# speechcatcher-asr/speechcatcher

Hardware: AMD Instinct MI355X
Metric: concurrent real-time streams (audio-seconds/s), de_xl dims, 640 ms (10240-sample) chunk steps, beam 10 CTC+attention (higher is better)
Workload: dtype f32

## Files before the change

include/scasr.h:

```cpp
#ifndef SCASR_H
#define SCASR_H

#include <stddef.h>
#include <stdint.h>

#ifdef __cplusplus
extern "C" {
#endif

#define SC_OK 0
#define SC_ERR_ARG (-1)
#define SC_ERR_LAUNCH (-2)
#define SC_ERR_CAPACITY (-3)
#define SC_ERR_INPUT (-4)

#define SC_GEMM_RELU 1
#define SC_GEMM_RESIDUAL 2
#define SC_GEMM_LN_AT_CROWS 8
#define SC_GEMM_NAIVE 4
#define SC_GEMM_SPLIT16 16

#define SC_F_ANY_EOS 1
#define SC_F_BEST_EOS 2
#define SC_F_ALL_EOS 4
// ... 494 lines not shown
int sc_conv1(const float *feat, int n_mels, const int32_t *jobs, int n_jobs, int max_t1,
             const float *w, const float *b, int d, float *c1, void *stream);

int sc_block_pack(const float *sub, const int32_t *jobs, int nb, int R, const float *pe, int d,
                  float *xblk, void *stream);

int sc_ctx_handoff(float *x, int R, const int32_t *jobs, int ns, float *state, int layer, int d,
                   void *stream);

int sc_enc_attention(const float *qkv, float *att, int nblk, int R, int H, int d, int masked,
                     void *stream);

int sc_encoder_layers(const sc_enc_layer *layers , int n_layers, float *x, int nblk, int R,
                      int masked, const int32_t *jobs, int ns, float *past_ctx, float *xn,
                      float *qkv, float *att, float *ffh, int d, int H, int F, float eps,
                      void *stream);


int sc_ctc_extend_state(const sc_search *sb , void *stream);
int sc_dec_embed(const sc_search *sb, void *stream);
int sc_kv_rows_to_half(const float *stage, const int32_t *rows, int m, int n_layers, int TCAP, int d2,
                       void *ckv_half, void *stream);
int sc_dec_self_attn(const sc_search *sb, int layer, void *stream);
int sc_dec_cross_attn(const sc_search *sb, int layer, void *stream);
int sc_decoder_layers(const sc_search *sb, void *stream);
#define SC_MAX_VOCAB 8192
int sc_logsoftmax_topk(const sc_search *sb, void *stream);
int sc_ctc_prefix_scan(const sc_search *sb, void *stream);
int sc_ctc_prefix_scan_split(const sc_search *sb, int split_min, void *stream);
int sc_fuse_topw(const sc_search *sb, void *stream);
int sc_beam_prune(const sc_search *sb, void *stream);
int sc_ctc_gather_state(const sc_search *sb, void *stream);
int sc_ctc_gather_state_split(const sc_search *sb, int split_min, void *stream);
int sc_decode_step(const sc_search *sb, void *stream);
int sc_decode_step_ex(const sc_search *sb, int scan_split_min, void *stream);
int sc_dec_layer_fused_supported(int d, int H, int W, int F);
int sc_dec_layer_self(const sc_search *sb, int layer, const float *x_in, float *x_out, const float *ffn_part,
                      int n_ffn_part, void *stream);
int sc_dec_layer_cross(const sc_search *sb, int layer, const float *x_in, float *x_out, void *stream);
int sc_dec_layer_ffn(const sc_search *sb, int layer, const float *x_in, float *x_out, float *ffn_part,
                     int max_part, int *n_part , void *stream);
int sc_dec_layer_stream_supported(int d, int H, int W, int F);
int sc_dec_layer_stream(const sc_search *sb, int layer, const float *x_in, float *x_out, float *xn_out,
                        const float *ffn_part, int n_ffn_part, void *stream);
int sc_dec_layer_ffn_xn(const sc_search *sb, int layer, const float *xn, float *ffn_part, int max_part,
                        int *n_part , void *stream);
int sc_dec_layer_reduce_ln(const sc_search *sb, int layer, const float *x_in, float *x_out, float *xn_out, void *stream);
int sc_dec_output_logits(const sc_search *sb, const float *x_in, float *x_out, const float *ffn_part,
                         int n_ffn_part, void *stream);


int sc_glu_dwconv_bn_swish(const float *y, int B, int T, int C, int ksize, const float *dw_w,
                           const float *dw_b, const float *bn_g, const float *bn_b,
                           const float *bn_mean, const float *bn_var, float bn_eps, float *out,
                           void *stream);

int sc_relpos_attention(const float *qkv, const float *p, const float *bias_u, const float *bias_v,
                        float *out, int B, int T, int H, int d, void *stream);
int sc_relpos_attention_masked(const float *qkv, const float *p, const float *bias_u, const float *bias_v,
                               float *out, int B, int T, int H, int d, const uint8_t *mask, int mask_mode,
                               void *stream);

typedef struct sc_config {
  int32_t d_model, enc_heads, enc_layers, dec_heads, dec_layers, ffn_dim, vocab_size;
  int32_t n_mels, n_fft, win_length, hop_length, sample_rate;
  int32_t block_size, hop_size, look_ahead, subsample, conv_freq1, conv_freq2;
// ... 135 lines not shown
```

speechcatcher_amd/_abi.py:

```python
import ctypes as C
import os
import subprocess
from pathlib import Path

HERE = Path(__file__).resolve().parent
LIB_PATH = HERE / "libscasr.so"
CSRC = HERE / "csrc"

c_float_p = C.POINTER(C.c_float)
c_int_p = C.POINTER(C.c_int32)
c_double_p = C.POINTER(C.c_double)
vp = C.c_void_p


class EncLayer(C.Structure):
    _fields_ = [(n, vp) for n in ("ln1_g", "ln1_b", "wqkv", "bqkv", "wo", "bo",
                                  "ln2_g", "ln2_b", "w1", "b1", "w2", "b2", "w1_p", "w2_p",
                                  "wqkv_p", "wo_p", "w1_h", "w2_h", "wqkv_h", "wo_h", "w1_s", "w2_s",
                                  "wqkv_s", "wo_s")]


class DecLayer(C.Structure):
    _fields_ = [(n, vp) for n in ("ln1_g", "ln1_b", "wqkv", "bqkv", "wo", "bo",
                                  "ln2_g", "ln2_b", "wq", "bq", "wo2", "bo2",
# ... 258 lines not shown
    "sc_prof_collect": (C.c_int, [c_double_p, c_double_p, C.POINTER(C.c_longlong)]),
    "sc_prof_collect2": (C.c_int, [c_double_p, c_double_p, c_double_p, C.POINTER(C.c_longlong)]),
    "sc_prof_event_overhead_ms": (C.c_double, [vp]),
    "sc_layernorm": (C.c_int, [vp, vp, C.c_int, vp, vp, C.c_int, C.c_int, C.c_int, vp, vp, C.c_float, vp]),
    "sc_copy_rows": (C.c_int, [vp, vp, vp, vp, C.c_int, C.c_int, vp]),
    "sc_log_softmax_rows": (C.c_int, [vp, vp, C.c_int, C.c_int, vp]),
    "sc_logmel": (C.c_int, [vp, C.c_int, vp, C.c_int, C.c_int, vp, vp, vp, vp, vp, C.c_int, C.c_int,
                            C.c_int, C.c_int, C.c_int, vp, vp]),
    "sc_conv1": (C.c_int, [vp, C.c_int, vp, C.c_int, C.c_int, vp, vp, C.c_int, vp, vp]),
    "sc_block_pack": (C.c_int, [vp, vp, C.c_int, C.c_int, vp, C.c_int, vp, vp]),
    "sc_ctx_handoff": (C.c_int, [vp, C.c_int, vp, C.c_int, vp, C.c_int, C.c_int, vp]),
    "sc_enc_attention": (C.c_int, [vp, vp, C.c_int, C.c_int, C.c_int, C.c_int, C.c_int, vp]),
    "sc_encoder_layers": (C.c_int, [vp, C.c_int, vp, C.c_int, C.c_int, C.c_int, vp, C.c_int, vp, vp,
                                    vp, vp, vp, C.c_int, C.c_int, C.c_int, C.c_float, vp]),
    "sc_glu_dwconv_bn_swish": (C.c_int, [vp, C.c_int, C.c_int, C.c_int, C.c_int, vp, vp, vp, vp, vp, vp,
                                         C.c_float, vp, vp]),
    "sc_relpos_attention": (C.c_int, [vp, vp, vp, vp, vp, C.c_int, C.c_int, C.c_int, C.c_int, vp]),
    "sc_relpos_attention_masked": (C.c_int, [vp, vp, vp, vp, vp, C.c_int, C.c_int, C.c_int, C.c_int, vp, C.c_int, vp]),
    "sc_ctc_extend_state": (C.c_int, [vp, vp]),
    "sc_dec_embed": (C.c_int, [vp, vp]),
    "sc_kv_rows_to_half": (C.c_int, [vp, vp, C.c_int, C.c_int, C.c_int, C.c_int, vp, vp]),
    "sc_dec_self_attn": (C.c_int, [vp, C.c_int, vp]),
    "sc_dec_cross_attn": (C.c_int, [vp, C.c_int, vp]),
    "sc_decoder_layers": (C.c_int, [vp, vp]),
    "sc_logsoftmax_topk": (C.c_int, [vp, vp]),
    "sc_ctc_prefix_scan": (C.c_int, [vp, vp]),
    "sc_fuse_topw": (C.c_int, [vp, vp]),
    "sc_beam_prune": (C.c_int, [vp, vp]),
    "sc_ctc_gather_state": (C.c_int, [vp, vp]),
    "sc_ctc_gather_state_split": (C.c_int, [vp, C.c_int, vp]),
    "sc_decode_step": (C.c_int, [vp, vp]),
    "sc_decode_step_ex": (C.c_int, [vp, C.c_int, vp]),
    "sc_ctc_prefix_scan_split": (C.c_int, [vp, C.c_int, vp]),
    "sc_dec_layer_fused_supported": (C.c_int, [C.c_int, C.c_int, C.c_int, C.c_int]),
    "sc_dec_layer_self": (C.c_int, [vp, C.c_int, vp, vp, vp, C.c_int, vp]),
    "sc_dec_layer_cross": (C.c_int, [vp, C.c_int, vp, vp, vp]),
    "sc_dec_layer_ffn": (C.c_int, [vp, C.c_int, vp, vp, vp, C.c_int, C.POINTER(C.c_int), vp]),
    "sc_dec_output_logits": (C.c_int, [vp, vp, vp, vp, C.c_int, vp]),
    "sc_streams_kv_rows": (C.c_int, [vp]),
    "sc_dec_layer_stream_supported": (C.c_int, [C.c_int, C.c_int, C.c_int, C.c_int]),
    "sc_dec_layer_stream": (C.c_int, [vp, C.c_int, vp, vp, vp, vp, C.c_int, vp]),
    "sc_dec_layer_reduce_ln": (C.c_int, [vp, C.c_int, vp, vp, vp, vp]),
    "sc_dec_layer_ffn_xn": (C.c_int, [vp, C.c_int, vp, vp, C.c_int, C.POINTER(C.c_int), vp]),
    "sc_engine_create": (C.c_int, [C.POINTER(Config), C.POINTER(NamedTensor), C.c_int, C.c_int, C.POINTER(vp)]),
    "sc_engine_load": (C.c_int, [C.c_char_p, C.c_int, C.POINTER(vp)]),
    "sc_engine_config": (C.c_int, [vp, C.POINTER(Config)]),
    "sc_engine_destroy": (None, [vp]),
    "sc_streams_create": (C.c_int, [vp, C.POINTER(StreamOptions), C.POINTER(vp)]),
    "sc_streams_destroy": (None, [vp]),
    "sc_push": (C.c_int, [vp, c_int_p, C.POINTER(vp), c_int_p, C.POINTER(C.c_uint8), C.c_int, c_int_p]),
    "sc_push_features": (C.c_int, [vp, c_int_p, C.POINTER(vp), c_int_p, C.POINTER(C.c_uint8), C.c_int, c_int_p]),
    "sc_get_hyps": (C.c_int, [vp, C.c_int, C.c_int, C.c_int, c_int_p, c_int_p, c_int_p, c_double_p, c_double_p,
                              c_double_p]),
    "sc_get_hyps_batch": (C.c_int, [vp, c_int_p, C.c_int, C.c_int, C.c_int, c_int_p, c_int_p, c_int_p, c_int_p,
                                    c_double_p, c_double_p, c_double_p]),
    "sc_submit": (C.c_int, [vp, c_int_p, C.POINTER(vp), c_int_p, C.POINTER(C.c_uint8), C.c_int]),
    "sc_poll": (C.c_int, [vp, C.c_int, C.c_int, c_int_p, c_int_p]),
    "sc_streams_outstanding": (C.c_int, [vp]),
    "sc_streams_set_encoder_batch": (C.c_int, [vp, C.c_int]),
    "sc_streams_set_queue_depth": (C.c_int, [vp, C.c_int]),
    "sc_stream_last_error": (C.c_char_p, [vp, C.c_int]),
    "sc_reset": (C.c_int, [vp, C.c_int]),
    "sc_stream_info": (C.c_int, [vp, C.c_int, C.POINTER(StreamInfo)]),
    "sc_streams_stats": (C.c_int, [vp, C.POINTER(C.c_long), C.POINTER(C.c_long), C.POINTER(C.c_long)]),
    "sc_streams_capture_stats": (C.c_int, [vp, C.POINTER(C.c_long), c_double_p]),
    "sc_streams_set_graphs": (C.c_int, [vp, C.c_int]),
# ... 138 lines not shown
```

speechcatcher_amd/csrc/search.hip:

```cpp
#include "common.h"
#include "attn.h"
#include <mutex>
#include <unordered_map>

#define SC_CTC_T(s) (CTRL(s, SC_C_TCTC) > 0 ? CTRL(s, SC_C_TCTC) : CTRL(s, SC_C_T))

#define XPOS(pp, s, h) (sb.xpos + (((long)(pp) * sb.S + (s)) * sb.W + (h)) * sb.LCAP)
#define CTCR(pp, s) (sb.ctc_r + ((long)(pp) * sb.S + (s)) * sb.TCAP * 2 * sb.W)
#define CTCRS(pp, s) (sb.ctc_rs + ((long)(pp) * sb.S + (s)) * sb.TCAP * sb.W)

__global__ void ctc_extend_state_kernel(sc_search sb) {
  const int s = blockIdx.x, h = threadIdx.x;
  if (!CTRL(s, SC_C_ACTIVE) || !CTRL(s, SC_C_HAS)) return;
  const int T = CTRL(s, SC_C_T), told = CTRL(s, SC_C_TOLD), nh = CTRL(s, SC_C_NHYP);
  if (h >= nh || told >= T) return;
  float *r = CTCR(CTRL(s, SC_C_CUR), s);
  float *rs = CTCRS(CTRL(s, SC_C_CUR), s);
  const float *x = sb.ctcx + (long)s * sb.TCAP * sb.V;
  const int t0 = told < 1 ? 1 : told;
  float rb = r[((long)(t0 - 1) * 2 + 1) * sb.W + h];
  for (int t = t0; t < T; ++t) {
    rb = rb + x[(long)t * sb.V + sb.blank];
    r[((long)t * 2 + 0) * sb.W + h] = SC_LOGZERO;
    r[((long)t * 2 + 1) * sb.W + h] = rb;
// ... 573 lines not shown
    float phi;
    ctc_frame(r_n, r_b, prs, pb, same, xc, xb, phi);
    if ((i & (SC_CTC_CK - 1)) == SC_CTC_CK - 1) {
      rn[((long)(t / SC_CTC_CK) * 2) * WK + e] = r_n;
      rn[((long)(t / SC_CTC_CK) * 2 + 1) * WK + e] = r_b;
    }
    ctc_psi_add(pm, ps, phi + xc);
    if (!has) cum += xb;
  };
  auto advance = [&](const CtcChunkT &q, int tb) {
    if (tb >= start && tb + 16 <= T) {
#pragma unroll
      for (int i = 0; i < 16; ++i) frame(q, tb, i);
    } else {
#pragma unroll
      for (int i = 0; i < 16; ++i)
        if (tb + i >= start && tb + i < T) frame(q, tb, i);
    }
  };
  if (start < T) {
    CtcChunkT qa, qb;
    int tb = start & ~15;
    fetch(qa, tb);
    while (true) {
      if (tb + 16 < T) fetch(qb, tb + 16);
      advance(qa, tb);
      tb += 16;
      if (tb >= T) break;
      if (tb + 16 < T) fetch(qa, tb + 16);
      advance(qb, tb);
      tb += 16;
      if (tb >= T) break;
    }
  }
  float psi = pm + logf(ps);
  const float rsum_last = has ? rsp[(long)(T - 1) * W + h] : cum;
  if (c == sb.eos) psi = rsum_last;
  if (c == sb.blank) psi = SC_LOGZERO;
  sb.psi[row * K + k] = psi;
  if (k == 0) sb.psi_eos[row] = rsum_last;
}

#define CTC_EB (256 / CTC_NSEG)
__global__ __launch_bounds__(256) void ctc_prefix_scan_tpar_kernel(sc_search sb, int split_min) {
  __shared__ float co[8][CTC_NSEG][CTC_EB];
  __shared__ float st0[2][CTC_NSEG][CTC_EB];
  __shared__ float cum0[CTC_NSEG][CTC_EB];
  const int s = blockIdx.y;
  if (!CTRL(s, SC_C_ACTIVE)) return;
  const int nh = CTRL(s, SC_C_NHYP), K = sb.K, W = sb.W, V = sb.V;
  const int T = SC_CTC_T(s), L = CTRL(s, SC_C_L), cur = CTRL(s, SC_C_CUR);
  if (!ctc_scan_is_split(T, L, split_min)) return;
  if ((int)blockIdx.x * CTC_EB >= nh * K) return;
  const int el = threadIdx.x % CTC_EB, p = threadIdx.x / CTC_EB;
  const int e_raw = blockIdx.x * CTC_EB + el;
  const bool valid = e_raw < nh * K;
  const int e = valid ? e_raw : nh * K - 1;
  const int h = e / K, k = e % K;
  const bool has = CTRL(s, SC_C_HAS);
  const long row = (long)s * W + h;
  const int c = sb.pre_ids[row * K + k];
  const int last = YSEQ(cur, s, h)[L - 1];
  const bool same = (c == last);
  const int tct = sb.tct;
  const float *__restrict__ xcol = sb.ctcxT + ((long)s * V + c) * tct;
  const float *__restrict__ xblk = sb.ctcxT + ((long)s * V + sb.blank) * tct;
// ... 91 lines not shown
    float n = r_n0, b = r_b0;
    float gm = r_n0, gs = 1.f;
    for (int q = 0; q < CTC_NSEG; ++q) {
      st0[0][q][el] = n;
      st0[1][q][el] = b;
      const float nn = lse2(co[0][q][el] + n, co[3][q][el]);
      const float nb = lse2(lse2(co[1][q][el] + n, co[2][q][el] + b), co[4][q][el]);
      n = nn;
      b = nb;
      const float m = sc_max_raw(gm, co[5][q][el]);
      gs = gs * sc_exp_neg(gm - m) + co[6][q][el] * sc_exp_neg(co[5][q][el] - m);
      gm = m;
    }
    if (valid) {
      float psi = gm + logf(gs);
      float total = 0.f;
      if (!has)
        for (int q = 0; q < CTC_NSEG; ++q) total += co[7][q][el];
      const float rsum_last = has ? rsp[(long)(T - 1) * W + h] : total;
      if (c == sb.eos) psi = rsum_last;
      if (c == sb.blank) psi = SC_LOGZERO;
      sb.psi[row * K + k] = psi;
      if (k == 0) sb.psi_eos[row] = rsum_last;
    }
  }
  __syncthreads();
  if (valid) {
    rn[((long)p * 2) * WK + e] = st0[0][p][el];
    rn[((long)p * 2 + 1) * WK + e] = st0[1][p][el];
  }
}

static std::mutex g_scan_split_mutex;
static std::unordered_map<const void *, int> g_scan_split;
static void scan_split_note(const sc_search *sbp, int eff) {
  std::lock_guard<std::mutex> lk(g_scan_split_mutex);
  g_scan_split[sbp->ctc_rnew] = eff;
}
static int scan_split_last(const sc_search *sbp) {
  std::lock_guard<std::mutex> lk(g_scan_split_mutex);
  auto it = g_scan_split.find(sbp->ctc_rnew);
  return it == g_scan_split.end() ? -1 : it->second;
}

extern "C" int sc_ctc_prefix_scan_split(const sc_search *sbp, int split_min, void *stream) {
  SC_CHECK_ARG(sbp, "null");
  SC_CHECK_ARG(sbp->ctcxT && sbp->tct >= 4 && sbp->tct % 4 == 0, "the prefix scan needs the column-major table copy (sc_search.ctcxT)");
  split_min = ctc_split_min_ok(sbp->TCAP, split_min);
  scan_split_note(sbp, split_min);
  dim3 grid(cdiv(sbp->W * sbp->K, 256), sbp->S);
  ctc_prefix_scan_colmajor_kernel<<<grid, 256, 0, (hipStream_t)stream>>>(*sbp, split_min);
  if (split_min > 0)
    ctc_prefix_scan_tpar_kernel<<<dim3(cdiv(sbp->W * sbp->K, CTC_EB), sbp->S), 256, 0, (hipStream_t)stream>>>(*sbp, split_min);
  SC_CHECK_LAUNCH();
  return SC_OK;
}

extern "C" int sc_ctc_prefix_scan(const sc_search *sbp, void *stream) { return sc_ctc_prefix_scan_split(sbp, 0, stream); }

__device__ __forceinline__ float sort_key_value(unsigned long long c) {
  unsigned u = (unsigned)(c >> 32);
  u = (u & 0x80000000u) ? (u & 0x7FFFFFFFu) : ~u;
  return __uint_as_float(u);
}

__global__ __launch_bounds__(256) void fuse_topw_kernel(sc_search sb) {
  extern __shared__ __attribute__((aligned(16))) float smem[];
  __shared__ int need_full;
  const int row = blockIdx.x, s = row / sb.W, h = row % sb.W;
  if (!CTRL(s, SC_C_ACTIVE) || h >= CTRL(s, SC_C_NHYP)) return;
  const int V = sb.V, K = sb.K, W = sb.W, tid = threadIdx.x;
  float *comb = smem, *ctc = smem + V;
  if (!(sb.w_ctc > 0.f)) {
    if (tid < W) {
      const int c = sb.pre_ids[(long)row * K + tid];
      sb.cand_tok[(long)row * W + tid] = c;
      sb.cand_score[(long)row * W + tid] = __fmul_rn(sb.w_dec, sb.logp[(long)row * V + c]);
      sb.cand_ctc[(long)row * W + tid] = 0.f;
    }
    return;
  }
  const float s_prev = CTRL(s, SC_C_HAS) ? sb.ctc_s[((long)CTRL(s, SC_C_CUR) * sb.S + s) * W + h] : 0.f;
  if (K < 64 && W <= 64 && sb.w_dec >= 0.f) {
    if (tid < 64) {
// ... 40 lines not shown
  }
  __syncthreads();
  for (int v = tid; v < V; v += 256) {
    const float cv = __fsub_rn(ctc[v], s_prev);
    ctc[v] = cv;
    comb[v] = __fadd_rn(__fmul_rn(sb.w_dec, sb.logp[(long)row * V + v]), __fmul_rn(sb.w_ctc, cv));
  }
  __syncthreads();
  const int NP = next_pow2(V);
  unsigned long long *comp = reinterpret_cast<unsigned long long *>(smem + 2 * V);
  for (int c = tid; c < NP; c += 256) comp[c] = c < V ? sort_key(comb[c], c) : 0ull;
  __syncthreads();
  block_bitonic_sort_desc(comp, NP);
  for (int k = tid; k < W; k += 256) {
    const int i = sort_key_index(comp[k]);
    sb.cand_tok[(long)row * W + k] = i;
    sb.cand_score[(long)row * W + k] = comb[i];
    sb.cand_ctc[(long)row * W + k] = ctc[i];
  }
}

extern "C" int sc_fuse_topw(const sc_search *sbp, void *stream) {
  SC_CHECK_ARG(sbp, "null");
  SC_CHECK_ARG(sbp->V > 0 && sbp->V <= SC_MAX_VOCAB, "vocabulary larger than SC_MAX_VOCAB (8192)");
  const size_t smem = fuse_topw_lds(sbp->V);
  const int rc = allow_large_lds(reinterpret_cast<const void *>(&fuse_topw_kernel), smem, fuse_topw_lds(SC_MAX_VOCAB),
                                 "sc_fuse_topw");
  if (rc != SC_OK) return rc;
  fuse_topw_kernel<<<sbp->S * sbp->W, 256, smem, (hipStream_t)stream>>>(*sbp);
  SC_CHECK_LAUNCH();
  return SC_OK;
}

__global__ __launch_bounds__(256) void beam_prune_kernel(sc_search sb) {
  extern __shared__ __attribute__((aligned(16))) double tot[];
  __shared__ int fl_any, fl_all, fl_best, fl_rep;
  __shared__ int win_h[64], win_tok[64];
  __shared__ unsigned bm[SC_KV_MAX_ROWS / 32];
  const int s = blockIdx.x, tid = threadIdx.x;
  if (!CTRL(s, SC_C_ACTIVE)) return;
  for (int w = tid; w < (sb.kv_rows + 31) / 32; w += 256) bm[w] = 0u;
  const int W = sb.W, K = sb.K;
  const int nh = CTRL(s, SC_C_NHYP), L = CTRL(s, SC_C_L), T = CTRL(s, SC_C_T);
  const int cur = CTRL(s, SC_C_CUR), o = 1 - cur;
  const int n = nh * W, nout = n < W ? n : W;
  if (tid == 0) { fl_any = 0; fl_all = 1; fl_best = 0; fl_rep = 0; }
  for (int e = tid; e < n; e += 256) {
    const int h = e / W, j = e % W;
    tot[e] = sb.score[((long)cur * sb.S + s) * W + h] + (double)sb.cand_score[((long)s * W + h) * W + j];
  }
  __syncthreads();
  for (int e = tid; e < n; e += 256) {
    const double te = tot[e];
    int rk = 0;
    for (int j = 0; j < n; ++j) rk += (tot[j] > te) || (tot[j] == te && j < e);
    if (rk >= nout) continue;
    const int h = e / W, j = e % W, i = rk;
    const long prow = (long)s * W + h;
    const int tok = sb.cand_tok[prow * W + j];
    win_h[i] = h;
    win_tok[i] = tok;
    const long oi = ((long)o * sb.S + s) * W + i, ci = ((long)cur * sb.S + s) * W + h;
    sb.score[oi] = te;
    sb.sc_dec[oi] = sb.sc_dec[ci] + (double)sb.logp[prow * sb.V + tok];
    sb.sc_ctc[oi] = sb.sc_ctc[ci] + (double)sb.cand_ctc[prow * W + j];
    int kk = -1;
    for (int q = 0; q < K; ++q)
      if (sb.pre_ids[prow * K + q] == tok) { kk = q; break; }
    float sval;
    if (tok == sb.blank) sval = SC_LOGZERO;
    else if (tok == sb.eos) sval = sb.psi_eos[prow];
    else if (kk >= 0) sval = sb.psi[prow * K + kk];
    else sval = SC_LOGZERO;
    sb.ctc_s[oi] = sval;
    sb.sel[((long)s * W + i) * 2] = h;
    sb.sel[((long)s * W + i) * 2 + 1] = kk < 0 ? 0 : kk;
    const bool is_eos = tok == sb.eos;
    if (is_eos) atomicOr(&fl_any, 1);
    else atomicAnd(&fl_all, 0);
    if (i == 0 && is_eos) atomicOr(&fl_best, 1);
  }
  __syncthreads();
  const int *asrc = ANC(cur, s);
  int *adst = ANC(o, s);
  bool rep = false;
  constexpr int UB = 4;
  const int ntot = nout * (L + 1);
  for (int e0 = tid; e0 < ntot; e0 += 256 * UB) {
    int yv[UB], xv[UB], av[UB];
#pragma unroll
    for (int u = 0; u < UB; ++u) {
      const int e = min(e0 + 256 * u, ntot - 1);
      const int i = e / (L + 1), p = min(e % (L + 1), L - 1);
      const int h = win_h[i];
      yv[u] = YSEQ(cur, s, h)[p];
      xv[u] = XPOS(cur, s, h)[p];
      av[u] = asrc[(long)p * W + h];
    }
#pragma unroll
    for (int u = 0; u < UB; ++u) {
      const int e = e0 + 256 * u;
      if (e >= ntot) break;
      const int i = e / (L + 1), p = e % (L + 1);
      const int tok = win_tok[i];
      int *ydst = YSEQ(o, s, i), *xdst = XPOS(o, s, i);
      if (p < L) {
        ydst[p] = yv[u];
        xdst[p] = xv[u];
        if (p >= 1 && yv[u] == tok && tok != sb.sos && tok != sb.eos) rep = true;
        adst[(long)p * W + i] = av[u];
        atomicOr(&bm[(av[u] >> 5) & (SC_KV_MAX_ROWS / 32 - 1)], 1u << (av[u] & 31));
      } else {
        ydst[L] = tok;
        xdst[L] = T - 1;
      }
    }
  }
  if (rep) atomicOr(&fl_rep, 1);
  __syncthreads();
  if (tid == 0)
    sb.flags[s] = (fl_any ? SC_F_ANY_EOS : 0) | (fl_best ? SC_F_BEST_EOS : 0) |
                  (fl_all ? SC_F_ALL_EOS : 0) | (fl_rep ? SC_F_REPEAT : 0);
  if (tid >= 64 || L + 1 > sb.LCAP) return;
  const int lane = tid, NR = sb.kv_rows, nwords = (NR + 31) / 32;
  int *out = adst + (long)L * W;
  int got = 0;
  for (int w0 = 0; w0 < nwords && got < nout; w0 += 64) {
    const int w = w0 + lane;
    unsigned fr = w < nwords ? ~bm[w] : 0u;
    if (w == nwords - 1 && (NR & 31)) fr &= (1u << (NR & 31)) - 1u;
    const int c = __popc(fr);
    int incl = c;
#pragma unroll
    for (int o2 = 1; o2 < 64; o2 <<= 1) {
      const int t = __shfl_up(incl, o2, 64);
      if (lane >= o2) incl += t;
    }
    int k = got + incl - c;
    while (fr && k < nout) {
      const int b = __ffs(fr) - 1;
      fr &= fr - 1u;
      out[k++] = w * 32 + b;
    }
    got += __shfl(incl, 63, 64);
  }
  if (got < nout && lane >= got && lane < nout) out[lane] = NR - 1;
  if (lane == 0 && sb.kvflags) sb.kvflags[s] = got < nout ? 1 : 0;
}

extern "C" int sc_beam_prune(const sc_search *sbp, void *stream) {
  SC_CHECK_ARG(sbp, "null");
  SC_CHECK_ARG(sbp->W <= 64, "beam wider than 64");
  SC_CHECK_ARG(sbp->kv_rows >= sbp->W && sbp->kv_rows <= SC_KV_MAX_ROWS, "kv_rows out of range (beam .. 65536)");
  size_t smem = (size_t)sbp->W * sbp->W * sizeof(double);
  beam_prune_kernel<<<sbp->S, 256, smem, (hipStream_t)stream>>>(*sbp);
  SC_CHECK_LAUNCH();
  return SC_OK;
}

__global__ __launch_bounds__(256) void ctc_gather_state_kernel(sc_search sb, int split_min) {
  const int s = blockIdx.y;
  if (!CTRL(s, SC_C_ACTIVE)) return;
  const int W = sb.W, K = sb.K, V = sb.V, T = SC_CTC_T(s), nh = CTRL(s, SC_C_NHYP), L = CTRL(s, SC_C_L);
  const int nout = nh * W < W ? nh * W : W;
  const int cur = CTRL(s, SC_C_CUR), o = 1 - cur;
  const bool has = CTRL(s, SC_C_HAS);
  const int WK = W * K, tct = sb.tct;
  float *dst = CTCR(o, s);
  float *dst_rs = CTCRS(o, s);
  const float *__restrict__ rp = CTCR(cur, s);
  const float *__restrict__ rsp = CTCRS(cur, s);
  const float *ck = sb.ctc_rnew + (long)s * ctc_tck(sb.TCAP) * 2 * WK;
  const int out_len = L - 1;
  int start = out_len > 1 ? out_len : 1;
  if (start > T) start = T;
  const bool split = ctc_scan_is_split(T, L, split_min);
  const int base = start & ~15;
  const int seg = split ? 16 * cdiv(T - base, 16 * CTC_NSEG) : SC_CTC_CK;
  const int nseg = split ? CTC_NSEG : cdiv(T, SC_CTC_CK);
  for (int idx = blockIdx.x * blockDim.x + threadIdx.x; idx < nout * nseg; idx += gridDim.x * blockDim.x) {
    const int i = idx % nout, j = idx / nout;
    const int h = sb.sel[((long)s * W + i) * 2], k = sb.sel[((long)s * W + i) * 2 + 1];
    const int e = h * K + k;
    const int c = sb.pre_ids[((long)s * W + h) * K + k];
    const bool same = c == YSEQ(cur, s, h)[L - 1];
    const float *__restrict__ xcol = sb.ctcxT + ((long)s * V + c) * tct;
    const float *__restrict__ xblk = sb.ctcxT + ((long)s * V + sb.blank) * tct;
    int t_lo, t_hi;
    float r_n, r_b;
    if (split) {
      t_lo = max(start, base + j * seg);
      t_hi = min(T, base + (j + 1) * seg);
      r_n = ck[((long)j * 2) * WK + e];
      r_b = ck[((long)j * 2 + 1) * WK + e];
      if (j == 0) {
        for (int t = 0; t < start - 1; ++t) {
// ... 38 lines not shown
      for (int q = 0; q < SC_CTC_CK / 4; ++q) {
        const int t4 = min(tb + 4 * q, tct - 4);
        const float4 c4 = *reinterpret_cast<const float4 *>(xcol + t4), b4 = *reinterpret_cast<const float4 *>(xblk + t4);
        xc[4 * q] = c4.x; xc[4 * q + 1] = c4.y; xc[4 * q + 2] = c4.z; xc[4 * q + 3] = c4.w;
        xb[4 * q] = b4.x; xb[4 * q + 1] = b4.y; xb[4 * q + 2] = b4.z; xb[4 * q + 3] = b4.w;
      }
#pragma unroll
      for (int q = 0; q < SC_CTC_CK; ++q) {
        const int tp = min(max(tb + q - 1, 0), T - 1);
        pn[q] = has ? rsp[(long)tp * W + h] : 0.f;
        pb[q] = has ? rp[((long)tp * 2 + 1) * W + h] : 0.f;
      }
#pragma unroll
      for (int q = 0; q < SC_CTC_CK; ++q) {
        const int t = tb + q;
        if (t >= t_lo && t < t_hi) {
          float phi;
          ctc_frame(r_n, r_b, has ? pn[q] : cum, has ? pb[q] : cum, same, xc[q], xb[q], phi);
          dst[((long)t * 2) * W + i] = r_n;
          dst[((long)t * 2 + 1) * W + i] = r_b;
          dst_rs[(long)t * W + i] = lse2(r_n, r_b);
          if (!has) cum += xb[q];
        }
      }
    }
  }
}

extern "C" int sc_ctc_gather_state_split(const sc_search *sbp, int split_min, void *stream) {
  SC_CHECK_ARG(sbp, "null");
  SC_CHECK_ARG(sbp->ctcxT && sbp->tct >= 4, "the state rebuild needs the column-major table copy (sc_search.ctcxT)");
  int gx = cdiv(ctc_tck(sbp->TCAP) * sbp->W, 256);
  if (gx > 16) gx = 16;
  const int eff = ctc_split_min_ok(sbp->TCAP, split_min), last = scan_split_last(sbp);
  if (last >= 0 && last != eff) {
    sc_set_error("sc_ctc_gather_state_split: the last prefix scan of this batch ran with split_min = %d, the rebuild was asked for %d - "
                 "streams split over T leave segment states, not checkpoints: pass the scan's value (sc_ctc_gather_state() = 0)", last, eff);
    return SC_ERR_ARG;
  }
  ctc_gather_state_kernel<<<dim3(gx, sbp->S), 256, 0, (hipStream_t)stream>>>(*sbp, eff);
  SC_CHECK_LAUNCH();
  return SC_OK;
}

extern "C" int sc_ctc_gather_state(const sc_search *sbp, void *stream) { return sc_ctc_gather_state_split(sbp, 0, stream); }

static bool dec_fused_ok(const sc_search &sb) {
  if (const char *e = sc_hook("SC_DEC_FUSED"))
    return atoi(e) != 0 && sc_dec_layer_fused_supported(sb.d, sb.H, sb.W, sb.F) && sb.ph1 && sb.out_w_q;
  if (const char *e = sc_hook("SC_FUSED_MAX"))
    if ((sb.rowmap ? sb.n_rows : sb.S * sb.W) > atoi(e) && sc_dec_layer_hpw(sb) < 2) return false;
  return sc_dec_layer_fused_supported(sb.d, sb.H, sb.W, sb.F) && sb.ph1 && sb.ph2 && sb.ffn_part &&
         sb.max_ffn_part >= 1 && sb.out_w_q && sb.V % sb.d == 0 && sb.layers && sb.layers[0].wqkv_pp &&
         sb.layers[0].wq_pp && sb.layers[0].wo_pp && sb.layers[0].w1_p;
}

int sc_decode_step_form(const sc_search *sbp) { return dec_fused_ok(*sbp) ? (sc_dec_layer_stream_form(*sbp) ? 2 : 1) : 0; }

extern "C" int sc_decode_step(const sc_search *sbp, void *stream) { return sc_decode_step_ex(sbp, 0, stream); }

extern "C" int sc_decode_step_ex(const sc_search *sbp, int scan_split_min, void *stream) {
  SC_CHECK_ARG(sbp, "null");
  const sc_search &sb = *sbp;
  const int n = sb.rowmap ? sb.n_rows : sb.S * sb.W;
  int rc;
  if (dec_fused_ok(sb) && sc_dec_layer_stream_form(sb)) {
    float *xa = sb.dx, *xb = sb.dxn;
    int npart = 0;
    for (int li = 0; li < sb.n_layers; ++li) {
      SC_TRY(sc_dec_layer_stream(sbp, li, xa, xb, sb.dq, sb.ffn_part, npart, stream));
      SC_TRY(sc_dec_layer_ffn_xn(sbp, li, sb.dq, sb.ffn_part, sb.max_ffn_part, &npart, stream));
      float *t = xa; xa = xb; xb = t;
    }
    SC_TRY(sc_dec_output_logits(sbp, xa, xb, sb.ffn_part, npart, stream));
  } else if (dec_fused_ok(sb)) {
    float *xa = sb.dx, *xb = sb.dxn;
    int npart = 0;
    for (int li = 0; li < sb.n_layers; ++li) {
      SC_TRY(sc_dec_layer_self(sbp, li, xa, xb, sb.ffn_part, npart, stream));
      SC_TRY(sc_dec_layer_cross(sbp, li, xb, xa, stream));
      if (sc_dec_layer_split_ffn(sb)) {
        SC_TRY(sc_dec_layer_reduce_ln(sbp, li, xa, xb, sb.dq, stream));
        SC_TRY(sc_dec_layer_ffn_xn(sbp, li, sb.dq, sb.ffn_part, sb.max_ffn_part, &npart, stream));
      } else
      SC_TRY(sc_dec_layer_ffn(sbp, li, xa, xb, sb.ffn_part, sb.max_ffn_part, &npart, stream));
      float *t = xa; xa = xb; xb = t;
    }
    SC_TRY(sc_dec_output_logits(sbp, xa, xb, sb.ffn_part, npart, stream));
  } else {
  SC_TRY(sc_dec_embed(sbp, stream));
  bool logits_done = false;
  SC_TRY(decoder_layers_impl(sbp, stream, true, &logits_done));
  if (!logits_done)
    SC_TRY(sc_gemm(sb.dxn, sb.rowmap, sb.d, sb.out_w, sb.out_b, sb.logits, sb.rowmap, sb.V, n, sb.V, sb.d, 0, 0, stream));
  }
  SC_TRY(sc_logsoftmax_topk(sbp, stream));
  const bool use_ctc = sb.w_ctc > 0.f;
  if (use_ctc) SC_TRY(sc_ctc_prefix_scan_split(sbp, scan_split_min, stream));
  SC_TRY(sc_fuse_topw(sbp, stream));
  SC_TRY(sc_beam_prune(sbp, stream));
  if (use_ctc) SC_TRY(sc_ctc_gather_state_split(sbp, scan_split_min, stream));
  return SC_OK;
}
```

speechcatcher_amd/hip_backend.py:

```python
import ctypes as C
import os
import warnings

import torch

from . import _abi


def _p(t):
    return 0 if t is None else t.data_ptr()


def resample(x, rate, device="cuda:0"):
    if not torch.cuda.is_available():
        raise _abi.ScasrError("resample needs a ROCm GPU (torch.cuda.is_available() is False)")
    lib = _abi.load()
    device = torch.device(device)
    x = torch.as_tensor(x).to(device, torch.float32).contiguous().reshape(-1)
    n_out = int(lib.sc_resample_out_count(int(rate), x.numel(), 1))
    if n_out < 0:
        _abi.check(n_out, "sc_resample_out_count")
    y = torch.empty(n_out, dtype=torch.float32, device=device)
    with torch.cuda.device(device):
        n = int(lib.sc_resample(_p(x), x.numel(), int(rate), _p(y), n_out, torch.cuda.current_stream(device).cuda_stream))
# ... 893 lines not shown

    def dec_layer_ffn(self, sb, li, xin, xout):
        n = C.c_int(0)
        self._sb_call("sc_dec_layer_ffn", sb, li, _p(xin), _p(xout), _p(sb.ffn_part), int(sb.ffn_part.shape[0]),
                      C.byref(n))
        return int(n.value)

    def dec_layer_stream(self, sb, li, xin, xout, xn_out, npart):
        self._sb_call("sc_dec_layer_stream", sb, li, _p(xin), _p(xout), _p(xn_out), _p(sb.ffn_part), int(npart))

    def dec_layer_ffn_xn(self, sb, li, xn):
        n = C.c_int(0)
        self._sb_call("sc_dec_layer_ffn_xn", sb, li, _p(xn), _p(sb.ffn_part), int(sb.ffn_part.shape[0]), C.byref(n))
        return int(n.value)

    def dec_output_logits(self, sb, xin, xout, npart):
        self._sb_call("sc_dec_output_logits", sb, _p(xin), _p(xout), _p(sb.ffn_part), int(npart))

    def logsoftmax_topk(self, sb):
        self._sb_call("sc_logsoftmax_topk", sb)

    def ctc_prefix_scan(self, sb, split_min=0):
        self._sb_call("sc_ctc_prefix_scan_split", sb, int(split_min))

    def fuse_topw(self, sb):
        self._sb_call("sc_fuse_topw", sb)

    def beam_prune(self, sb):
        self._sb_call("sc_beam_prune", sb)

    def ctc_gather_state(self, sb, split_min=0):
        self._sb_call("sc_ctc_gather_state_split", sb, int(split_min))

    def decode_step(self, sb):
        if not self.use_graphs:
            self._sb_call("sc_decode_step", sb)
            return
        graphs = getattr(sb, "_sc_decode_graphs", None)
        if graphs is None:
            graphs = sb._sc_decode_graphs = {}
        g = graphs.get(int(sb.n_rows_step))
        st = self._stream()
        if g is None:
            if st == 0:
                raise _abi.ScasrError("hipGraph capture needs a non-default stream (StreamBatch.stream)")
            self._sb_call("sc_decode_step", sb)
            self._chk(self.lib.sc_graph_capture_begin(st), "sc_graph_capture_begin")
            try:
                self._sb_call("sc_decode_step", sb)
            finally:
                out = C.c_void_p()
                rc = self.lib.sc_graph_capture_end(st, C.byref(out))
            self._chk(rc, "sc_graph_capture_end")
            graphs[int(sb.n_rows_step)] = out
            return self._redo_after_capture(sb)
        self._chk(self.lib.sc_graph_launch(g, st), "sc_graph_launch")

    def prepare_decode(self, sb):
        if not self.use_graphs or self._stream() == 0:
            return
        keep = sb.n_rows_step
        for nb in range(sb.row_bucket, sb.S + sb.row_bucket, sb.row_bucket):
            sb.n_rows_step = min(nb, sb.S) * sb.W
            if int(sb.n_rows_step) not in getattr(sb, "_sc_decode_graphs", {}):
                self.decode_step(sb)
        sb.n_rows_step = keep
# ... 4 lines not shown
```

Baseline: 4055.

## Compute CTC prefix psi only and rebuild state for winning hypotheses inside beam prune

The prefix scan now computes only the psi scores for all W*K candidates and no longer writes per-frame checkpoint states. After pruning, the CTC forward variables are recomputed only for the W surviving hypotheses, using a 64-thread wave that stages frames through shared memory. This wave is fused into the beam-prune kernel as an extra wave, and a separate gather kernel runs only for streams split over T. The aim is to avoid writing and gathering state for every candidate, at the cost of walking the winners' frames a second time and a larger, more complex prune kernel.

Result: no change. 4075 (median of 4 runs) (+0.5%).

```diff
diff --git a/include/scasr.h b/include/scasr.h
--- a/include/scasr.h
+++ b/include/scasr.h
@@ -550,6 +550,9 @@
 int sc_beam_prune(const sc_search *sb, void *stream);
 int sc_ctc_gather_state(const sc_search *sb, void *stream);
 int sc_ctc_gather_state_split(const sc_search *sb, int split_min, void *stream);
+int sc_ctc_prefix_psi_split(const sc_search *sb, int split_min, void *stream);
+int sc_ctc_rebuild_winners_split(const sc_search *sb, int split_min, void *stream);
+int sc_beam_prune_rebuild_split(const sc_search *sb, int split_min, void *stream);
 int sc_decode_step(const sc_search *sb, void *stream);
 int sc_decode_step_ex(const sc_search *sb, int scan_split_min, void *stream);
 int sc_dec_layer_fused_supported(int d, int H, int W, int F);
diff --git a/speechcatcher_amd/_abi.py b/speechcatcher_amd/_abi.py
--- a/speechcatcher_amd/_abi.py
+++ b/speechcatcher_amd/_abi.py
@@ -314,6 +314,9 @@
     "sc_decode_step": (C.c_int, [vp, vp]),
     "sc_decode_step_ex": (C.c_int, [vp, C.c_int, vp]),
     "sc_ctc_prefix_scan_split": (C.c_int, [vp, C.c_int, vp]),
+    "sc_ctc_prefix_psi_split": (C.c_int, [vp, C.c_int, vp]),
+    "sc_ctc_rebuild_winners_split": (C.c_int, [vp, C.c_int, vp]),
+    "sc_beam_prune_rebuild_split": (C.c_int, [vp, C.c_int, vp]),
     "sc_dec_layer_fused_supported": (C.c_int, [C.c_int, C.c_int, C.c_int, C.c_int]),
     "sc_dec_layer_self": (C.c_int, [vp, C.c_int, vp, vp, vp, C.c_int, vp]),
     "sc_dec_layer_cross": (C.c_int, [vp, C.c_int, vp, vp, vp]),
diff --git a/speechcatcher_amd/csrc/search.hip b/speechcatcher_amd/csrc/search.hip
--- a/speechcatcher_amd/csrc/search.hip
+++ b/speechcatcher_amd/csrc/search.hip
@@ -629,6 +629,104 @@
       tb += 16;
       if (tb >= T) break;
     }
+  }
+  float psi = pm + logf(ps);
+  const float rsum_last = has ? rsp[(long)(T - 1) * W + h] : cum;
+  if (c == sb.eos) psi = rsum_last;
+  if (c == sb.blank) psi = SC_LOGZERO;
+  sb.psi[row * K + k] = psi;
+  if (k == 0) sb.psi_eos[row] = rsum_last;
+}
+
+template <bool HAS>
+struct CtcPsiChunkT {
+  float4 xc[4];
+  float4 xb[HAS ? 1 : 4];
+  float ph[HAS ? 16 : 1];
+};
+template <bool HAS>
+__device__ __forceinline__ void ctc_psi_walk(const float *__restrict__ xcol, const float *__restrict__ xblk,
+                                             const float *__restrict__ pp, int pstep, int tct, int start, int T, float &pm,
+                                             float &ps, float &cum) {
+  auto fetch = [&](CtcPsiChunkT<HAS> &q, int tb) {
+#pragma unroll
+    for (int j = 0; j < 4; ++j) {
+      const int t4 = min(tb + 4 * j, tct - 4);
+      q.xc[j] = *reinterpret_cast<const float4 *>(xcol + t4);
+      if (!HAS) q.xb[j] = *reinterpret_cast<const float4 *>(xblk + t4);
+    }
+    if (HAS) {
+#pragma unroll
+      for (int i = 0; i < 16; ++i) {
+        int t = tb + i;
+        t = t < T ? (t < 1 ? 1 : t) : T - 1;
+        q.ph[i] = pp[(t - 1) * pstep];
+      }
+    }
+  };
+  auto frame = [&](const CtcPsiChunkT<HAS> &q, int i) {
+    const float4 c4 = q.xc[i >> 2];
+    const float xc = (i & 3) == 0 ? c4.x : (i & 3) == 1 ? c4.y : (i & 3) == 2 ? c4.z : c4.w;
+    const float phi = HAS ? q.ph[HAS ? i : 0] : cum;
+    ctc_psi_add(pm, ps, phi + xc);
+    if (!HAS) {
+      const float4 b4 = q.xb[HAS ? 0 : i >> 2];
+      cum += (i & 3) == 0 ? b4.x : (i & 3) == 1 ? b4.y : (i & 3) == 2 ? b4.z : b4.w;
+    }
+  };
+  auto advance = [&](const CtcPsiChunkT<HAS> &q, int tb) {
+    if (tb >= start && tb + 16 <= T) {
+#pragma unroll
+      for (int i = 0; i < 16; ++i) frame(q, i);
+    } else {
+#pragma unroll
+      for (int i = 0; i < 16; ++i)
+        if (tb + i >= start && tb + i < T) frame(q, i);
+    }
+  };
+  CtcPsiChunkT<HAS> qa, qb;
+  int tb = start & ~15;
+  const int npair = (T - tb + 31) >> 5;
+  fetch(qa, tb);
+  for (int it = 0; it < npair; ++it) {
+    fetch(qb, tb + 16);
+    advance(qa, tb);
+    fetch(qa, tb + 32);
+    advance(qb, tb + 16);
+    tb += 32;
+  }
+}
+
+__global__ __launch_bounds__(256) void ctc_prefix_psi_kernel(sc_search sb, int split_min) {
+  const int s = blockIdx.y;
+  if (!CTRL(s, SC_C_ACTIVE)) return;
+  const int nh = CTRL(s, SC_C_NHYP), K = sb.K, W = sb.W, V = sb.V;
+  const int e = blockIdx.x * 256 + threadIdx.x;
+  if (e >= nh * K) return;
+  const int h = e / K, k = e % K;
+  const int T = SC_CTC_T(s), L = CTRL(s, SC_C_L), cur = CTRL(s, SC_C_CUR);
+  if (ctc_scan_is_split(T, L, split_min)) return;
+  const bool has = CTRL(s, SC_C_HAS);
+  const long row = (long)s * W + h;
+  const int c = sb.pre_ids[row * K + k];
+  const int last = YSEQ(cur, s, h)[L - 1];
+  const bool same = (c == last);
+  const int tct = sb.tct;
+  const float *__restrict__ xcol = sb.ctcxT + ((long)s * V + c) * tct;
+  const float *__restrict__ xblk = sb.ctcxT + ((long)s * V + sb.blank) * tct;
+  const float *__restrict__ rsp = CTCRS(cur, s);
+  const float *__restrict__ pp = same ? CTCR(cur, s) + W + h : rsp + h;
+  const int pstep = same ? 2 * W : W;
+  const int out_len = L - 1;
+  int start = out_len > 1 ? out_len : 1;
+  if (start > T) start = T;
+  float cum = 0.f;
+  if (!has)
+    for (int t = 0; t < start; ++t) cum += xblk[t];
+  float pm = (out_len == 0) ? xcol[0] : SC_LOGZERO, ps = 1.f;
+  if (start < T) {
+    if (has) ctc_psi_walk<true>(xcol, xblk, pp, pstep, tct, start, T, pm, ps, cum);
+    else ctc_psi_walk<false>(xcol, xblk, pp, pstep, tct, start, T, pm, ps, cum);
   }
   float psi = pm + logf(ps);
   const float rsum_last = has ? rsp[(long)(T - 1) * W + h] : cum;
@@ -786,24 +884,39 @@
 }
 
 static std::mutex g_scan_split_mutex;
-static std::unordered_map<const void *, int> g_scan_split;
-static void scan_split_note(const sc_search *sbp, int eff) {
+struct ScanSplitNote { int eff; bool psi_only; };
+static std::unordered_map<const void *, ScanSplitNote> g_scan_split;
+static void scan_split_note(const sc_search *sbp, int eff, bool psi_only) {
   std::lock_guard<std::mutex> lk(g_scan_split_mutex);
-  g_scan_split[sbp->ctc_rnew] = eff;
-}
-static int scan_split_last(const sc_search *sbp) {
+  g_scan_split[sbp->ctc_rnew] = ScanSplitNote{eff, psi_only};
+}
+static int scan_split_last(const sc_search *sbp, bool *psi_only = nullptr) {
   std::lock_guard<std::mutex> lk(g_scan_split_mutex);
   auto it = g_scan_split.find(sbp->ctc_rnew);
-  return it == g_scan_split.end() ? -1 : it->second;
+  if (psi_only) *psi_only = it != g_scan_split.end() && it->second.psi_only;
+  return it == g_scan_split.end() ? -1 : it->second.eff;
 }
 
 extern "C" int sc_ctc_prefix_scan_split(const sc_search *sbp, int split_min, void *stream) {
   SC_CHECK_ARG(sbp, "null");
   SC_CHECK_ARG(sbp->ctcxT && sbp->tct >= 4 && sbp->tct % 4 == 0, "the prefix scan needs the column-major table copy (sc_search.ctcxT)");
   split_min = ctc_split_min_ok(sbp->TCAP, split_min);
-  scan_split_note(sbp, split_min);
+  scan_split_note(sbp, split_min, false);
   dim3 grid(cdiv(sbp->W * sbp->K, 256), sbp->S);
   ctc_prefix_scan_colmajor_kernel<<<grid, 256, 0, (hipStream_t)stream>>>(*sbp, split_min);
+  if (split_min > 0)
+    ctc_prefix_scan_tpar_kernel<<<dim3(cdiv(sbp->W * sbp->K, CTC_EB), sbp->S), 256, 0, (hipStream_t)stream>>>(*sbp, split_min);
+  SC_CHECK_LAUNCH();
+  return SC_OK;
+}
+
+extern "C" int sc_ctc_prefix_psi_split(const sc_search *sbp, int split_min, void *stream) {
+  SC_CHECK_ARG(sbp, "null");
+  SC_CHECK_ARG(sbp->ctcxT && sbp->tct >= 4 && sbp->tct % 4 == 0, "the prefix scan needs the column-major table copy (sc_search.ctcxT)");
+  split_min = ctc_split_min_ok(sbp->TCAP, split_min);
+  scan_split_note(sbp, split_min, true);
+  dim3 grid(cdiv(sbp->W * sbp->K, 256), sbp->S);
+  ctc_prefix_psi_kernel<<<grid, 256, 0, (hipStream_t)stream>>>(*sbp, split_min);
   if (split_min > 0)
     ctc_prefix_scan_tpar_kernel<<<dim3(cdiv(sbp->W * sbp->K, CTC_EB), sbp->S), 256, 0, (hipStream_t)stream>>>(*sbp, split_min);
   SC_CHECK_LAUNCH();
@@ -910,18 +1023,20 @@
   return SC_OK;
 }
 
-__global__ __launch_bounds__(256) void beam_prune_kernel(sc_search sb) {
+template <bool EXTRA, typename Walk>
+__device__ __forceinline__ void beam_prune_body(const sc_search &sb, Walk walk) {
   extern __shared__ __attribute__((aligned(16))) double tot[];
   __shared__ int fl_any, fl_all, fl_best, fl_rep;
   __shared__ int win_h[64], win_tok[64];
   __shared__ unsigned bm[SC_KV_MAX_ROWS / 32];
   const int s = blockIdx.x, tid = threadIdx.x;
   if (!CTRL(s, SC_C_ACTIVE)) return;
-  for (int w = tid; w < (sb.kv_rows + 31) / 32; w += 256) bm[w] = 0u;
+  const int npr = (!EXTRA || tid < 256) ? 256 : 0;
   const int W = sb.W, K = sb.K;
   const int nh = CTRL(s, SC_C_NHYP), L = CTRL(s, SC_C_L), T = CTRL(s, SC_C_T);
   const int cur = CTRL(s, SC_C_CUR), o = 1 - cur;
-  const int n = nh * W, nout = n < W ? n : W;
+  const int n = npr ? nh * W : 0, nout = nh * W < W ? nh * W : W;
+  for (int w = tid; npr && w < (sb.kv_rows + 31) / 32; w += 256) bm[w] = 0u;
   if (tid == 0) { fl_any = 0; fl_all = 1; fl_best = 0; fl_rep = 0; }
   for (int e = tid; e < n; e += 256) {
     const int h = e / W, j = e % W;
@@ -963,7 +1078,8 @@
   int *adst = ANC(o, s);
   bool rep = false;
   constexpr int UB = 4;
-  const int ntot = nout * (L + 1);
+  const int ntot = npr ? nout * (L + 1) : 0;
+  if (EXTRA && !npr) walk();
   for (int e0 = tid; e0 < ntot; e0 += 256 * UB) {
     int yv[UB], xv[UB], av[UB];
 #pragma unroll
@@ -1026,6 +1142,10 @@
   if (lane == 0 && sb.kvflags) sb.kvflags[s] = got < nout ? 1 : 0;
 }
 
+__global__ __launch_bounds__(256) void beam_prune_kernel(sc_search sb) {
+  beam_prune_body<false>(sb, [] {});
+}
+
 extern "C" int sc_beam_prune(const sc_search *sbp, void *stream) {
   SC_CHECK_ARG(sbp, "null");
   SC_CHECK_ARG(sbp->W <= 64, "beam wider than 64");
@@ -1036,10 +1156,11 @@
   return SC_OK;
 }
 
-__global__ __launch_bounds__(256) void ctc_gather_state_kernel(sc_search sb, int split_min) {
+__global__ __launch_bounds__(256) void ctc_gather_state_kernel(sc_search sb, int split_min, int split_only) {
   const int s = blockIdx.y;
   if (!CTRL(s, SC_C_ACTIVE)) return;
   const int W = sb.W, K = sb.K, V = sb.V, T = SC_CTC_T(s), nh = CTRL(s, SC_C_NHYP), L = CTRL(s, SC_C_L);
+  if (split_only && !ctc_scan_is_split(T, L, split_min)) return;
   const int nout = nh * W < W ? nh * W : W;
   const int cur = CTRL(s, SC_C_CUR), o = 1 - cur;
   const bool has = CTRL(s, SC_C_HAS);
@@ -1144,18 +1265,214 @@
   SC_CHECK_ARG(sbp->ctcxT && sbp->tct >= 4, "the state rebuild needs the column-major table copy (sc_search.ctcxT)");
   int gx = cdiv(ctc_tck(sbp->TCAP) * sbp->W, 256);
   if (gx > 16) gx = 16;
-  const int eff = ctc_split_min_ok(sbp->TCAP, split_min), last = scan_split_last(sbp);
+  bool psi_only = false;
+  const int eff = ctc_split_min_ok(sbp->TCAP, split_min), last = scan_split_last(sbp, &psi_only);
   if (last >= 0 && last != eff) {
     sc_set_error("sc_ctc_gather_state_split: the last prefix scan of this batch ran with split_min = %d, the rebuild was asked for %d - "
                  "streams split over T leave segment states, not checkpoints: pass the scan's value (sc_ctc_gather_state() = 0)", last, eff);
     return SC_ERR_ARG;
   }
-  ctc_gather_state_kernel<<<dim3(gx, sbp->S), 256, 0, (hipStream_t)stream>>>(*sbp, eff);
+  if (psi_only) {
+    sc_set_error("sc_ctc_gather_state_split: the last prefix scan of this batch was sc_ctc_prefix_psi_split, which leaves no "
+                 "checkpoints for the streams it walks: rebuild the state with sc_ctc_rebuild_winners_split");
+    return SC_ERR_ARG;
+  }
+  ctc_gather_state_kernel<<<dim3(gx, sbp->S), 256, 0, (hipStream_t)stream>>>(*sbp, eff, 0);
   SC_CHECK_LAUNCH();
   return SC_OK;
 }
 
 extern "C" int sc_ctc_gather_state(const sc_search *sbp, void *stream) { return sc_ctc_gather_state_split(sbp, 0, stream); }
+
+struct CtcWinChunkT {
+  float4 xc[4], xb[4];
+  float ph[16];
+};
+#define CTC_WIN_MAXW 32
+#define CTC_WIN_RS (SC_CTC_CK * 2 * CTC_WIN_MAXW)
+#define CTC_WIN_SINK (CTC_WIN_RS + SC_CTC_CK * CTC_WIN_MAXW)
+struct CtcWinStage { float f[CTC_WIN_SINK + 2 * CTC_WIN_MAXW]; };
+template <int NIT>
+__device__ __forceinline__ void ctc_rebuild_winners_stream(const sc_search &sb, int s, int tid, CtcWinStage &st) {
+  constexpr int nthr = 64;
+  const int W = sb.W, K = sb.K, V = sb.V, T = SC_CTC_T(s), nh = CTRL(s, SC_C_NHYP), L = CTRL(s, SC_C_L);
+  const int nout = nh * W < W ? nh * W : W;
+  const int cur = CTRL(s, SC_C_CUR), o = 1 - cur;
+  const bool has = CTRL(s, SC_C_HAS);
+  const int tct = sb.tct;
+  if (T < 1 || nout < 1) return;
+  float *dst = CTCR(o, s);
+  float *dst_rs = CTCRS(o, s);
+  const int out_len = L - 1;
+  int start = out_len > 1 ? out_len : 1;
+  if (start > T) start = T;
+  const bool isb = tid & 1;
+  const bool live = (tid >> 1) < nout;
+  const int i = live ? tid >> 1 : nout - 1;
+  const int h = sb.sel[((long)s * W + i) * 2], k = sb.sel[((long)s * W + i) * 2 + 1];
+  const int c = sb.pre_ids[((long)s * W + h) * K + k];
+  const bool same = c == YSEQ(cur, s, h)[L - 1];
+  const float *__restrict__ xcol = sb.ctcxT + ((long)s * V + c) * tct;
+  const float *__restrict__ xblk = sb.ctcxT + ((long)s * V + sb.blank) * tct;
+  const float *__restrict__ pp = same ? CTCR(cur, s) + W + h : CTCRS(cur, s) + h;
+  const int pstep = same ? 2 * W : W;
+  float r_n = (out_len == 0) ? xcol[0] : SC_LOGZERO;
+  float r_b = SC_LOGZERO;
+  const float r_first = isb ? r_b : r_n;
+  const int sink = CTC_WIN_SINK + (tid & (2 * CTC_WIN_MAXW - 1));
+  const int st_r = live ? (isb ? W : 0) + i : sink, st_r_step = live ? 2 * W : 0;
+  const int st_rs = live && isb ? CTC_WIN_RS + i : sink, st_rs_step = live && isb ? W : 0;
+  float cum = 0.f;
+  if (!has)
+    for (int t = 0; t < start; ++t) cum += xblk[t];
+
+  auto fetch = [&](CtcWinChunkT &q, int tb) {
+#pragma unroll
+    for (int j = 0; j < 4; ++j) {
+      const int t4 = min(tb + 4 * j, tct - 4);
+      q.xc[j] = *reinterpret_cast<const float4 *>(xcol + t4);
+      q.xb[j] = *reinterpret_cast<const float4 *>(xblk + t4);
+    }
+#pragma unroll
+    for (int q16 = 0; q16 < 16; ++q16) {
+      int t = tb + q16;
+      t = t < T ? (t < 1 ? 1 : t) : T - 1;
+      q.ph[q16] = pp[(t - 1) * pstep];
+    }
+  };
+  auto stage_sync = [] {
+    __builtin_amdgcn_fence(__ATOMIC_RELEASE, "wavefront");
+    __builtin_amdgcn_wave_barrier();
+    __builtin_amdgcn_fence(__ATOMIC_ACQUIRE, "wavefront");
+  };
+  auto frame = [&](const CtcWinChunkT &q, int j) {
+    const float4 c4 = q.xc[j >> 2], b4 = q.xb[j >> 2];
+    const float xc = (j & 3) == 0 ? c4.x : (j & 3) == 1 ? c4.y : (j & 3) == 2 ? c4.z : c4.w;
+    const float xb = (j & 3) == 0 ? b4.x : (j & 3) == 1 ? b4.y : (j & 3) == 2 ? b4.z : b4.w;
+    const float phi = has ? q.ph[j] : cum;
+    const float v = lse2(r_n, isb ? r_b : phi);
+    const float nr = v + (isb ? xb : xc);
+    st.f[st_rs + j * st_rs_step] = v;
+    st.f[st_r + j * st_r_step] = nr;
+    const float other = dpp_mov<SC_DPP_XOR1>(nr);
+    r_n = isb ? other : nr;
+    r_b = nr;
+    if (!has) cum += xb;
+  };
+  auto advance = [&](const CtcWinChunkT &q, int tb) {
+    if (tb >= start && tb + 16 <= T) {
+#pragma unroll
+      for (int j = 0; j < 16; ++j) frame(q, j);
+    } else {
+#pragma unroll
+      for (int j = 0; j < 16; ++j)
+        if (tb + j >= start && tb + j < T) frame(q, j);
+    }
+    const int lo = max(tb, start), hi = min(tb + 16, T);
+    const int n_r = (hi - lo) * 2 * W, n_rs = (hi - lo) * W;
+    float *const g_r = dst + (long)lo * 2 * W, *const g_rs = dst_rs + (long)(lo - 1) * W;
+    const int l_r = (lo - tb) * 2 * W, l_rs = CTC_WIN_RS + (lo - tb) * W;
+    stage_sync();
+#pragma unroll
+    for (int u = 0; u < NIT; ++u) {
+      const int idx = min(tid + u * nthr, n_r - 1);
+      g_r[idx] = st.f[l_r + idx];
+    }
+#pragma unroll
+    for (int u = 0; u < (NIT + 1) / 2; ++u) {
+      const int idx = min(tid + u * nthr, n_rs - 1);
+      g_rs[idx] = st.f[l_rs + idx];
+    }
+    stage_sync();
+  };
+  if (start < T) {
+    CtcWinChunkT qa, qb;
+    int tb = start & ~15;
+    fetch(qa, tb);
+    while (true) {
+      fetch(qb, tb + 16);
+      advance(qa, tb);
+      tb += 16;
+      if (tb >= T) break;
+      fetch(qa, tb + 16);
+      advance(qb, tb);
+      tb += 16;
+      if (tb >= T) break;
+    }
+  }
+  if (live && isb) dst_rs[(long)(T - 1) * W + i] = lse2(r_n, r_b);
+  if (live) dst[((long)(start - 1) * 2 + (isb ? 1 : 0)) * W + i] = r_first;
+  const float lz2 = lse2(SC_LOGZERO, SC_LOGZERO);
+  for (int idx = tid; idx < (start - 1) * W; idx += nthr) {
+    dst[(long)idx * 2] = SC_LOGZERO;
+    dst[(long)idx * 2 + 1] = SC_LOGZERO;
+    dst_rs[idx] = lz2;
+  }
+}
+
+template <int NIT>
+__global__ __launch_bounds__(64) void ctc_rebuild_winners_kernel(sc_search sb, int split_min) {
+  __shared__ CtcWinStage st;
+  const int s = blockIdx.x;
+  if (!CTRL(s, SC_C_ACTIVE)) return;
+  if (ctc_scan_is_split(SC_CTC_T(s), CTRL(s, SC_C_L), split_min)) return;
+  ctc_rebuild_winners_stream<NIT>(sb, s, threadIdx.x, st);
+}
+
+template <int NIT>
+__global__ __launch_bounds__(320) void beam_prune_rebuild_kernel(sc_search sb, int split_min) {
+  __shared__ CtcWinStage st;
+  beam_prune_body<true>(sb, [&] {
+    const int s = blockIdx.x;
+    if (ctc_scan_is_split(SC_CTC_T(s), CTRL(s, SC_C_L), split_min)) return;
+    ctc_rebuild_winners_stream<NIT>(sb, s, threadIdx.x - 256, st);
+  });
+}
+
+static int rebuild_winners_args(const sc_search *sbp, int split_min, const char *who) {
+  if (!sbp || !(sbp->ctcxT && sbp->tct >= 4 && sbp->tct % 4 == 0) || !(sbp->W >= 1 && sbp->W <= 16)) {
+    sc_set_error("%s: null batch, no column-major table copy (sc_search.ctcxT) or a beam wider than 16", who);
+    return -1;
+  }
+  const int eff = ctc_split_min_ok(sbp->TCAP, split_min), last = scan_split_last(sbp);
+  if (last >= 0 && last != eff) {
+    sc_set_error("%s: the last prefix scan of this batch ran with split_min = %d, the rebuild was asked for %d - "
+                 "the scan and the rebuild must agree on which streams were split over T: pass the scan's value", who, last, eff);
+    return -1;
+  }
+  return eff;
+}
+static void gather_split_streams(const sc_search *sbp, int eff, void *stream) {
+  int gx = cdiv(ctc_tck(sbp->TCAP) * sbp->W, 256);
+  if (gx > 16) gx = 16;
+  ctc_gather_state_kernel<<<dim3(gx, sbp->S), 256, 0, (hipStream_t)stream>>>(*sbp, eff, 1);
+}
+
+extern "C" int sc_ctc_rebuild_winners_split(const sc_search *sbp, int split_min, void *stream) {
+  const int eff = rebuild_winners_args(sbp, split_min, "sc_ctc_rebuild_winners_split");
+  if (eff < 0) return SC_ERR_ARG;
+  const int nit = cdiv(2 * SC_CTC_CK * sbp->W, 64);
+  if (nit <= 3) ctc_rebuild_winners_kernel<3><<<sbp->S, 64, 0, (hipStream_t)stream>>>(*sbp, eff);
+  else if (nit <= 5) ctc_rebuild_winners_kernel<5><<<sbp->S, 64, 0, (hipStream_t)stream>>>(*sbp, eff);
+  else ctc_rebuild_winners_kernel<8><<<sbp->S, 64, 0, (hipStream_t)stream>>>(*sbp, eff);
+  if (eff > 0) gather_split_streams(sbp, eff, stream);
+  SC_CHECK_LAUNCH();
+  return SC_OK;
+}
+
+extern "C" int sc_beam_prune_rebuild_split(const sc_search *sbp, int split_min, void *stream) {
+  const int eff = rebuild_winners_args(sbp, split_min, "sc_beam_prune_rebuild_split");
+  if (eff < 0) return SC_ERR_ARG;
+  SC_CHECK_ARG(sbp->kv_rows >= sbp->W && sbp->kv_rows <= SC_KV_MAX_ROWS, "kv_rows out of range (beam .. 65536)");
+  const size_t smem = (size_t)sbp->W * sbp->W * sizeof(double);
+  const int nit = cdiv(2 * SC_CTC_CK * sbp->W, 64);
+  if (nit <= 3) beam_prune_rebuild_kernel<3><<<sbp->S, 320, smem, (hipStream_t)stream>>>(*sbp, eff);
+  else if (nit <= 5) beam_prune_rebuild_kernel<5><<<sbp->S, 320, smem, (hipStream_t)stream>>>(*sbp, eff);
+  else beam_prune_rebuild_kernel<8><<<sbp->S, 320, smem, (hipStream_t)stream>>>(*sbp, eff);
+  if (eff > 0) gather_split_streams(sbp, eff, stream);
+  SC_CHECK_LAUNCH();
+  return SC_OK;
+}
 
 static bool dec_fused_ok(const sc_search &sb) {
   if (const char *e = sc_hook("SC_DEC_FUSED"))
@@ -1208,9 +1525,9 @@
   }
   SC_TRY(sc_logsoftmax_topk(sbp, stream));
   const bool use_ctc = sb.w_ctc > 0.f;
-  if (use_ctc) SC_TRY(sc_ctc_prefix_scan_split(sbp, scan_split_min, stream));
+  if (use_ctc) SC_TRY(sc_ctc_prefix_psi_split(sbp, scan_split_min, stream));
   SC_TRY(sc_fuse_topw(sbp, stream));
-  SC_TRY(sc_beam_prune(sbp, stream));
-  if (use_ctc) SC_TRY(sc_ctc_gather_state_split(sbp, scan_split_min, stream));
+  if (use_ctc) SC_TRY(sc_beam_prune_rebuild_split(sbp, scan_split_min, stream));
+  else SC_TRY(sc_beam_prune(sbp, stream));
   return SC_OK;
 }
diff --git a/speechcatcher_amd/hip_backend.py b/speechcatcher_amd/hip_backend.py
--- a/speechcatcher_amd/hip_backend.py
+++ b/speechcatcher_amd/hip_backend.py
@@ -949,6 +949,15 @@
     def ctc_gather_state(self, sb, split_min=0):
         self._sb_call("sc_ctc_gather_state_split", sb, int(split_min))
 
+    def ctc_prefix_psi(self, sb, split_min=0):
+        self._sb_call("sc_ctc_prefix_psi_split", sb, int(split_min))
+
+    def ctc_rebuild_winners(self, sb, split_min=0):
+        self._sb_call("sc_ctc_rebuild_winners_split", sb, int(split_min))
+
+    def beam_prune_rebuild(self, sb, split_min=0):
+        self._sb_call("sc_beam_prune_rebuild_split", sb, int(split_min))
+
     def decode_step(self, sb):
         if not self.use_graphs:
             self._sb_call("sc_decode_step", sb)
```
